# yemam3/SAC-RCBF

Measured on AMD Instinct MI355X. Metric: safe env steps/sec (dynamics+CBF-QP) at batch 65536, 1/2/4/8 MI355X, higher is better.
Workload: dtype f32 rows / f64 QP / f64 env

## Files before the change

__graft_entry__.py:

```python
import os
import subprocess
import sys

ROOT = os.path.dirname(os.path.abspath(__file__))
PKG = os.path.join(ROOT, "sac-rcbf_amd")
CSRC = os.path.join(PKG, "csrc")
LIB = os.path.join(PKG, "rcbf_amd", "librcbf_hip.so")
HIPCC = os.environ.get("HIPCC", "/opt/rocm/bin/hipcc")
HIP_FLAGS = ["--offload-arch=gfx950", "-O3", "-fPIC", "-std=c++17",
             "-fhip-fp32-correctly-rounded-divide-sqrt", "-Wno-unused-result",
             "-mllvm", "-amdgpu-kernarg-preload-count=16"]

for p in (ROOT, PKG):
    if p not in sys.path:
        sys.path.insert(0, p)


def _newer(target, sources):
    if not os.path.exists(target):
        return False
    t = os.path.getmtime(target)
    return all(os.path.getmtime(s) <= t for s in sources)


KERNEL_TUS = ["rcbf_qp.hip", "rcbf_qp_f64.hip", "rcbf_qp_bwd.hip", "rcbf_layer.hip", "rcbf_env.hip", "rcbf_cascade.hip",
              "rcbf_gp.hip", "rcbf_model.hip", "rcbf_aql.hip", "rcbf_steps_traj.hip", "rcbf_steps_term.hip"]
TU_FLAGS = {"rcbf_steps_term.hip": ["-mllvm", "-disable-machine-licm"]}
LLVM_BIN = "/opt/rocm/lib/llvm/bin"
STEPS_CO = os.path.join(PKG, "rcbf_amd", "librcbf_steps.co")
STEPS_TRAJ_CO = os.path.join(PKG, "rcbf_amd", "librcbf_steps_traj.co")
STEPS_TERM_CO = os.path.join(PKG, "rcbf_amd", "librcbf_steps_term.co")


def _deps(path, seen=None):
    import re
    seen = set() if seen is None else seen
    if path in seen or not os.path.exists(path):
        return seen
    seen.add(path)
    for name in re.findall(r'^\s*#\s*include\s+"([^"]+)"', open(path).read(), re.M):
        for d in (os.path.dirname(path), CSRC, os.path.join(ROOT, "include")):
            cand = os.path.normpath(os.path.join(d, name))
            if os.path.exists(cand):
                _deps(cand, seen)
                break
    return seen
# ... 13 lines not shown
        src = os.path.join(CSRC, tu)
        obj = os.path.join(objdir, tu.replace(".hip", ".o"))
        objs.append(obj)
        if not force and _newer(obj, sorted(_deps(src))):
            continue
        cmd = [HIPCC, *HIP_FLAGS, *TU_FLAGS.get(tu, []), *defines, *inc, "-c", "-o", obj, src]
        print("[build]", " ".join(cmd), flush=True)
        procs.append(subprocess.Popen(cmd))
    if any(p.wait() != 0 for p in procs):
        raise RuntimeError("hipcc failed")
    open(flags_file, "w").write(flags)
    if out == LIB:
        extract_steps_co(os.path.join(objdir, "rcbf_env.o"), STEPS_CO)
        extract_steps_co(os.path.join(objdir, "rcbf_steps_traj.o"), STEPS_TRAJ_CO)
        extract_steps_co(os.path.join(objdir, "rcbf_steps_term.o"), STEPS_TERM_CO)
    if not procs and _newer(out, objs):
        return out
    cmd = [HIPCC, "--offload-arch=gfx950", "-shared", "-fPIC", "-o", out, *objs, "-L/opt/rocm/lib", "-lhsa-runtime64"]
    print("[build]", " ".join(cmd), flush=True)
    subprocess.run(cmd, check=True)
    return out


def extract_steps_co(obj, out):
    if _newer(out, [obj]):
        return out
    import tempfile
    with tempfile.TemporaryDirectory() as td:
        fat = os.path.join(td, "fatbin.bin")
        subprocess.run([os.path.join(LLVM_BIN, "llvm-objcopy"), "--dump-section=.hip_fatbin=" + fat, obj,
# ... 139 lines not shown
    torch.cuda.synchronize()
    print("[smoke] ok", flush=True)


if __name__ == "__main__":
    what = sys.argv[1] if len(sys.argv) > 1 else "build"
    if what == "variant":
        name, defs = sys.argv[2], sys.argv[3:]
        os.makedirs(os.path.join(ROOT, "build", "variants"), exist_ok=True)
        vdir = os.path.join(ROOT, "build", "variants")
        build_lib(force=True, out=os.path.join(vdir, f"librcbf_{name}.so"), defines=defs)
        objdir = os.path.join(ROOT, "build", "obj_" + "_".join(d.strip("-D").replace("=", "") for d in defs))
        extract_steps_co(os.path.join(objdir, "rcbf_env.o"), os.path.join(vdir, f"librcbf_{name}.co"))
        extract_steps_co(os.path.join(objdir, "rcbf_steps_traj.o"), os.path.join(vdir, f"librcbf_{name}_traj.co"))
        extract_steps_co(os.path.join(objdir, "rcbf_steps_term.o"), os.path.join(vdir, f"librcbf_{name}_term.co"))
    else:
        {"build": build, "smoke": smoke, "build_oracle": lambda: build_oracle(force=True)}[what]()
```

include/rcbf_hip.h:

```cpp
#ifndef RCBF_HIP_H
#define RCBF_HIP_H

#include <stdint.h>
#include <hip/hip_runtime_api.h>

#ifdef __cplusplus
extern "C" {
#endif

#define RCBF_ABI_VERSION 13

#define RCBF_MODE_SIMULATED_CARS 0
#define RCBF_MODE_UNICYCLE 1

#define RCBF_FORM_DIFF 0
#define RCBF_FORM_CASCADE 1

#define RCBF_SOLVER_ACTIVE_SET 0
#define RCBF_SOLVER_PDIPM 1
#define RCBF_SOLVER_GI 2

#define RCBF_QP_OK 0
#define RCBF_QP_MAX_ITER 1
#define RCBF_QP_INFEASIBLE 2
// ... 221 lines not shown
#define RCBF_TRAJ_U 2
#define RCBF_TRAJ_REWARD 4
#define RCBF_TRAJ_COST 8
#define RCBF_TRAJ_DONE 16
#define RCBF_TRAJ_GOAL_MET 32
#define RCBF_TRAJ_STATUS 64
#define RCBF_TRAJ_TERM_OBS 128
#define RCBF_AQL_PROFILE 1
#define RCBF_AQL_FIRST_ACQUIRE_SYSTEM 2
#define RCBF_AQL_LAST_RELEASE_AGENT 4
#define RCBF_AQL_STUDY_MID_NOFENCE 8
#define RCBF_AQL_STUDY_MID_NOACQ 16
#define RCBF_AQL_STUDY_MID_NOREL 32
#define RCBF_AQL_PROFILE_ENDS 64
#define RCBF_AQL_PER_STEP 128
#define RCBF_AQL_SAFE_STEP_KERNARG_BYTES 408
#define RCBF_AQL_SAFE_STEPS_KERNARG_BYTES 408
#define RCBF_AQL_SAFE_STEPS_TRAJ_KERNARG_BYTES 424
#define RCBF_AQL_SAFE_STEPS_TERM_KERNARG_BYTES 432
typedef struct rcbf_aql rcbf_aql;
typedef struct rcbf_aql_plan rcbf_aql_plan;
int rcbf_aql_open(int32_t device, const char* code_object, int32_t flags, rcbf_aql** out);
int rcbf_aql_close(rcbf_aql* q);
int rcbf_aql_kernel_count(const rcbf_aql* q);
int rcbf_aql_safe_step_plan(rcbf_aql* q, const rcbf_params* prm, int64_t B, int32_t K, double* x, double* aux,
                            int32_t* step, uint32_t* episode, const float* const* u_rl_seq, int32_t n_u_rl,
                            const float* mu, const float* sigma, int32_t prior_cols, float* obs_out, float* u_out,
                            float* reward, float* cost, uint8_t* done, uint8_t* goal_met, int32_t* status_out,
                            int32_t* fail_flag, int32_t auto_reset, uint64_t seed, int64_t env_offset,
                            uint64_t* span_out, int32_t flags, rcbf_aql_plan** out);
// ... 2 lines not shown
                                 const float* mu, const float* sigma, int32_t prior_cols, float* obs_out,
                                 float* u_out, float* reward, float* cost, uint8_t* done, uint8_t* goal_met,
                                 int32_t* status_out, int32_t* fail_flag, int32_t auto_reset, uint64_t seed,
                                 int64_t env_offset, uint64_t* span_out, int32_t flags, int32_t traj_mask,
                                 int64_t traj_pitch, rcbf_aql_plan** out);
int rcbf_aql_safe_step_term_plan(rcbf_aql* q, const rcbf_params* prm, int64_t B, int32_t K, double* x, double* aux,
                                 int32_t* step, uint32_t* episode, const float* const* u_rl_seq, int32_t n_u_rl,
                                 const float* mu, const float* sigma, int32_t prior_cols, float* obs_out,
                                 float* u_out, float* reward, float* cost, uint8_t* done, uint8_t* goal_met,
                                 int32_t* status_out, int32_t* fail_flag, int32_t auto_reset, uint64_t seed,
                                 int64_t env_offset, uint64_t* span_out, int32_t flags, int32_t traj_mask,
                                 int64_t traj_pitch, float* term_obs, rcbf_aql_plan** out);
int rcbf_aql_run(rcbf_aql_plan* plan, uint64_t timeout_us);
int rcbf_aql_plan_times(const rcbf_aql_plan* plan, uint64_t* start_end_ns);
int rcbf_aql_plan_dispatches(const rcbf_aql_plan* plan);
int rcbf_aql_plan_free(rcbf_aql_plan* plan);

const char* rcbf_version(void);
int32_t rcbf_abi_version(void);
int32_t rcbf_params_size(void);

#ifdef __cplusplus
}
#endif
#endif
```

sac-rcbf_amd/csrc/rcbf_aql.hip:

```cpp
#include <hip/hip_runtime.h>
#include <hsa/hsa.h>
#include <hsa/hsa_ext_amd.h>

#include <dlfcn.h>
#include <immintrin.h>
#include <time.h>

#include <atomic>
#include <cstddef>
#include <cstdio>
#include <cstring>
#include <string>
#include <vector>

#include "rcbf_hip.h"
#include "rcbf_safe_step.hpp"

namespace {

using namespace rcbf;

struct SafeStepArgs {
    int64_t B;
    double* x;
// ... 49 lines not shown

}

struct rcbf_aql {
    int device = -1;
    hsa_agent_t agent{};
    hsa_queue_t* queue = nullptr;
    hsa_code_object_reader_t reader{};
    hsa_code_object_reader_t reader_traj{};
    hsa_executable_t exe{};
    hsa_executable_t exe_traj{};
    hsa_code_object_reader_t reader_term{};
    hsa_executable_t exe_term{};
    bool have_reader = false, have_reader_traj = false, have_exe = false, have_exe_traj = false, hsa_up = false;
    bool have_reader_term = false, have_exe_term = false;
    std::vector<char> code, code_traj, code_term;
    std::vector<KernelInfo> kernels;
    std::atomic<int> queue_error{0};
    int profiling = 0;
    bool fused = false;
    bool traj = false;
    bool term = false;
};

struct rcbf_aql_plan {
    rcbf_aql* q = nullptr;
    int device = -1;
    int32_t K = 0;
    void* kernargs = nullptr;
    std::vector<hsa_kernel_dispatch_packet_t> pkt;
    std::vector<hsa_signal_t> sig;
    int profiled = 0;
};

namespace {

void queue_error_cb(hsa_status_t status, hsa_queue_t*, void* data) {
    auto* q = static_cast<rcbf_aql*>(data);
    q->queue_error.store((int)status);
}

struct AgentSearch {
    uint32_t bdf;
    uint32_t domain;
    hsa_agent_t found{};
    bool ok = false;
};
// ... 49 lines not shown
    return buf;
}

std::string safe_steps_traj_prefix(int mode, int k, int bs) {
    char buf[128];
    snprintf(buf, sizeof buf, "_ZN4rcbf17k_safe_steps_trajILi%dELi%dELi%dEEEv", mode, k, bs);
    return buf;
}

std::string safe_steps_term_prefix(int mode, int k, int bs) {
    char buf[128];
    snprintf(buf, sizeof buf, "_ZN4rcbf17k_safe_steps_termILi%dELi%dELi%dEEEv", mode, k, bs);
    return buf;
}

bool read_side_code_object(const std::string& path, const char* suffix, std::vector<char>& code) {
    if (path.size() <= 3 || path.compare(path.size() - 3, 3, ".co") != 0) return true;
    const std::string tpath = path.substr(0, path.size() - 3) + suffix + ".co";
    FILE* tf = fopen(tpath.c_str(), "rb");
    if (!tf) return true;
    fseek(tf, 0, SEEK_END);
    const long tn = ftell(tf);
    fseek(tf, 0, SEEK_SET);
    code.resize(tn > 0 ? (size_t)tn : 0);
    const bool ok = tn > 0 && fread(code.data(), 1, (size_t)tn, tf) == (size_t)tn;
    fclose(tf);
    return ok;
}

template <typename T>
// ... 23 lines not shown
    explicit DeviceGuard(int dev) {
        if (hipGetDevice(&prev) != hipSuccess) prev = -1;
        if (prev != dev) (void)hipSetDevice(dev);
    }
    ~DeviceGuard() {
        if (prev >= 0) (void)hipSetDevice(prev);
    }
};

void destroy(rcbf_aql* q) {
    if (!q) return;
    if (q->queue) hsa_queue_destroy(q->queue);
    if (q->have_exe) hsa_executable_destroy(q->exe);
    if (q->have_exe_traj) hsa_executable_destroy(q->exe_traj);
    if (q->have_exe_term) hsa_executable_destroy(q->exe_term);
    if (q->have_reader) hsa_code_object_reader_destroy(q->reader);
    if (q->have_reader_traj) hsa_code_object_reader_destroy(q->reader_traj);
    if (q->have_reader_term) hsa_code_object_reader_destroy(q->reader_term);
    if (q->hsa_up) hsa_shut_down();
    delete q;
}

}

extern "C" {

int rcbf_aql_open(int32_t device, const char* code_object_path, int32_t flags, rcbf_aql** out) {
    if (!out) return RCBF_E_NULL;
    *out = nullptr;
    int ndev = 0;
    if (hipGetDeviceCount(&ndev) != hipSuccess || device < 0 || device >= ndev) return RCBF_E_BAD_SHAPE;
    std::string path;
    if (code_object_path && *code_object_path) {
// ... 13 lines not shown
    fseek(f, 0, SEEK_END);
    const long n = ftell(f);
    fseek(f, 0, SEEK_SET);
    q->code.resize(n > 0 ? (size_t)n : 0);
    const bool read_ok = n > 0 && fread(q->code.data(), 1, (size_t)n, f) == (size_t)n;
    fclose(f);
    if (!read_ok) {
        delete q;
        return RCBF_E_BAD_SHAPE;
    }
    if (!read_side_code_object(path, "_traj", q->code_traj)) {
        delete q;
        return RCBF_E_BAD_SHAPE;
    }
    if (!read_side_code_object(path, "_term", q->code_term)) {
        delete q;
        return RCBF_E_BAD_SHAPE;
    }
    int rc = hsa_rc(hsa_init());
    if (rc) {
        delete q;
        return rc;
    }
    q->hsa_up = true;
    hipDeviceProp_t prop;
    if (hipGetDeviceProperties(&prop, device) != hipSuccess) {
        destroy(q);
        return RCBF_E_HSA;
    }
    AgentSearch s{(uint32_t)((prop.pciBusID << 8) | (prop.pciDeviceID << 3)), (uint32_t)prop.pciDomainID};
// ... 28 lines not shown
    }
    if (!rc && !q->code_term.empty()) {
        rc = hsa_rc(
            hsa_code_object_reader_create_from_memory(q->code_term.data(), q->code_term.size(), &q->reader_term));
        if (!rc) q->have_reader_term = true;
        if (!rc)
            rc = hsa_rc(hsa_executable_create_alt(HSA_PROFILE_FULL, HSA_DEFAULT_FLOAT_ROUNDING_MODE_DEFAULT, nullptr,
                                                  &q->exe_term));
        if (!rc) q->have_exe_term = true;
        if (!rc)
            rc = hsa_rc(
                hsa_executable_load_agent_code_object(q->exe_term, q->agent, q->reader_term, nullptr, nullptr));
        if (!rc) rc = hsa_rc(hsa_executable_freeze(q->exe_term, nullptr));
        if (!rc) rc = hsa_rc(hsa_executable_iterate_agent_symbols(q->exe_term, q->agent, collect_kernel, q));
    }
    int n_steps = 0, n_fused = 0, n_traj = 0, n_term = 0;
    for (const auto& k : q->kernels) {
        if (k.name.compare(0, 21, "_ZN4rcbf11k_safe_step") == 0) {
            ++n_steps;
            if (k.kernarg_bytes != sizeof(SafeStepArgs) || k.private_bytes != 0) rc = RCBF_E_BAD_SHAPE;
        } else if (k.name.compare(0, 22, "_ZN4rcbf12k_safe_steps") == 0) {
            ++n_fused;
            if (k.kernarg_bytes != sizeof(SafeStepsArgs) || k.private_bytes != 0) rc = RCBF_E_BAD_SHAPE;
        } else if (k.name.compare(0, 27, "_ZN4rcbf17k_safe_steps_traj") == 0) {
            ++n_traj;
            if (k.kernarg_bytes != sizeof(SafeStepsTrajArgs) || k.private_bytes != 0) rc = RCBF_E_BAD_SHAPE;
        } else if (k.name.compare(0, 27, "_ZN4rcbf17k_safe_steps_term") == 0) {
            ++n_term;
            if (k.kernarg_bytes != sizeof(SafeStepsTermArgs) || k.private_bytes != 0) rc = RCBF_E_BAD_SHAPE;
        }
    }
    if (!rc && n_steps == 0) rc = RCBF_E_BAD_MODE;
    q->fused = n_fused > 0;
    q->traj = n_traj > 0;
    q->term = n_term > 0;
    if (!rc)
        rc = hsa_rc(hsa_queue_create(q->agent, kQueueSize, HSA_QUEUE_TYPE_SINGLE, queue_error_cb, q, UINT32_MAX,
                                     UINT32_MAX, &q->queue));
    if (!rc && q->profiling) rc = hsa_rc(hsa_amd_profiling_set_profiler_enabled(q->queue, 1));
    if (rc) {
        destroy(q);
        return rc;
    }
    *out = q;
    return 0;
}

int rcbf_aql_close(rcbf_aql* q) {
    destroy(q);
    return 0;
// ... 82 lines not shown
                       {reward, ext(row_rew, n * 4)},
                       {cost, ext(row_cost, n * 4)},
                       {done, ext(row_done, n)},
                       {goal_met, ext(row_goal, n)},
                       {status_out, ext(row_stat, n * 4)},
                       {term_obs, ext(row_term, 0)},
                       {fail_flag, 4}};
        for (int32_t j = 0; j < n_u_rl && kf; ++j)
            for (const auto& w : written)
                if (overlaps(u_rl_seq[j], nu * n * 4, w.p, w.bytes)) {
                    kf = nullptr;
                    break;
                }
    }
    if (term && !kf) return RCBF_E_BAD_MODE;
    const int32_t npkt = kf ? (K + kFusedChunk - 1) / kFusedChunk : K;

    auto* p = new rcbf_aql_plan();
    p->q = q;
    p->device = q->device;
    p->K = K;
    p->profiled = ends ? 2 : profiled ? 1 : 0;
    const size_t table_off = (size_t)npkt * kArgStride;
    std::vector<unsigned char> host(table_off + (kf ? (size_t)n_u_rl * sizeof(const float*) : 0), 0);
    int rc = (int)hipMalloc(&p->kernargs, host.size());
    if (kf) std::memcpy(host.data() + table_off, u_rl_seq, (size_t)n_u_rl * sizeof(const float*));
    for (int32_t j = 0; j < npkt && !rc; ++j) {
        const int64_t r0 = kf ? (int64_t)j * kFusedChunk : (int64_t)j;
        if (kf) {
            SafeStepsTermArgs ea;
            std::memset(&ea, 0, sizeof ea);
            SafeStepsTrajArgs& ta = ea.t;
            SafeStepsArgs& a = ta.s;
            ea.term_obs = rows_on(term_obs, r0, row_term);
            ta.traj_mask = traj_mask;
            ta.traj_pitch = traj_pitch;
            a.B = B;
// ... 49 lines not shown
        a.stamp_buf = span_out ? reinterpret_cast<unsigned long long*>(span_out) + (size_t)j * 4 * ((B + 63) / 64)
                               : nullptr;
        std::memcpy(host.data() + (size_t)j * kArgStride, &a, sizeof a);
    }
    if (!rc) rc = (int)hipMemcpy(p->kernargs, host.data(), host.size(), hipMemcpyHostToDevice);
    const int nsig = p->profiled == 1 ? npkt : p->profiled == 2 ? (npkt > 1 ? 2 : 1) : 1;
    for (int j = 0; !rc && j < nsig; ++j) {
        hsa_signal_t s;
        rc = hsa_rc(hsa_signal_create(1, 0, nullptr, &s));
        if (!rc) p->sig.push_back(s);
    }
    if (rc) {
        rcbf_aql_plan_free(p);
        return rc;
    }
    const KernelInfo* kd = kf ? kf : ki;
    p->pkt.resize(npkt);
    for (int32_t j = 0; j < npkt; ++j) {
        hsa_kernel_dispatch_packet_t& d = p->pkt[j];
        std::memset(&d, 0, sizeof d);
        int acq = j == 0 && (flags & RCBF_AQL_FIRST_ACQUIRE_SYSTEM) ? HSA_FENCE_SCOPE_SYSTEM : HSA_FENCE_SCOPE_AGENT;
        int rel =
            j == npkt - 1 && !(flags & RCBF_AQL_LAST_RELEASE_AGENT) ? HSA_FENCE_SCOPE_SYSTEM : HSA_FENCE_SCOPE_AGENT;
        if ((flags & (RCBF_AQL_STUDY_MID_NOFENCE | RCBF_AQL_STUDY_MID_NOACQ)) && j > 0) acq = HSA_FENCE_SCOPE_NONE;
        if ((flags & (RCBF_AQL_STUDY_MID_NOFENCE | RCBF_AQL_STUDY_MID_NOREL)) && j < npkt - 1)
            rel = HSA_FENCE_SCOPE_NONE;
        d.header = (uint16_t)((HSA_PACKET_TYPE_KERNEL_DISPATCH << HSA_PACKET_HEADER_TYPE) |
                              (1 << HSA_PACKET_HEADER_BARRIER) | (acq << HSA_PACKET_HEADER_SCACQUIRE_FENCE_SCOPE) |
                              (rel << HSA_PACKET_HEADER_SCRELEASE_FENCE_SCOPE));
        d.setup = (uint16_t)(1 << HSA_KERNEL_DISPATCH_PACKET_SETUP_DIMENSIONS);
        d.workgroup_size_x = (uint16_t)bs;
        d.workgroup_size_y = 1;
        d.workgroup_size_z = 1;
        d.grid_size_x = (uint32_t)(groups * (uint64_t)bs);
        d.grid_size_y = 1;
        d.grid_size_z = 1;
        d.private_segment_size = kd->private_bytes;
        d.group_segment_size = kd->group_bytes;
        d.kernel_object = kd->object;
        d.kernarg_address = static_cast<unsigned char*>(p->kernargs) + (size_t)j * kArgStride;
        if (p->profiled == 1)
            d.completion_signal = p->sig[j];
        else if (p->profiled == 2 && (j == 0 || j == npkt - 1))
            d.completion_signal = j == 0 ? p->sig.front() : p->sig.back();
        else if (j == npkt - 1)
            d.completion_signal = p->sig[0];
        else
            d.completion_signal.handle = 0;
    }
// ... 106 lines not shown
            start_end_ns[2 * j] = start_end_ns[2 * j + 1] = 0;
            if (j != 0 && j != p->K - 1) continue;
            sg = j == 0 ? p->sig.front() : p->sig.back();
        } else {
            sg = p->sig[j];
        }
        if (hsa_amd_profiling_get_dispatch_time(p->q->agent, sg, &t) != HSA_STATUS_SUCCESS) return RCBF_E_HSA;
        start_end_ns[2 * j] = (uint64_t)((long double)t.start * 1e9L / (long double)freq);
        start_end_ns[2 * j + 1] = (uint64_t)((long double)t.end * 1e9L / (long double)freq);
    }
    return 0;
}

int rcbf_aql_plan_dispatches(const rcbf_aql_plan* p) { return p ? (int)p->pkt.size() : RCBF_E_NULL; }

int rcbf_aql_plan_free(rcbf_aql_plan* p) {
    if (!p) return 0;
    if (p->kernargs) {
        DeviceGuard guard(p->device);
        (void)hipFree(p->kernargs);
    }
    for (auto& s : p->sig) hsa_signal_destroy(s);
    delete p;
    return 0;
}

}
```

sac-rcbf_amd/rcbf_amd/_lib.py:

```python
import ctypes
import os
import warnings

import torch

_HERE = os.path.dirname(os.path.abspath(__file__))
LIB_PATH = os.environ.get("RCBF_HIP_LIB", os.path.join(_HERE, "librcbf_hip.so"))

MODE_SIMULATED_CARS = 0
MODE_UNICYCLE = 1
FORM_DIFF = 0
FORM_CASCADE = 1
SOLVER_ACTIVE_SET = 0
SOLVER_PDIPM = 1
SOLVER_GI = 2
QP_OK, QP_MAX_ITER, QP_INFEASIBLE, QP_NONFINITE = 0, 1, 2, 3
MAX_HAZARDS = 8
ABI_VERSION = 13

_ERRORS = {1001: "RCBF_E_BAD_MODE", 1002: "RCBF_E_BAD_SHAPE", 1003: "RCBF_E_NULL", 1004: "RCBF_E_HSA",
           1005: "RCBF_E_TIMEOUT", 1006: "RCBF_E_GP_HANDOFF"}


class RcbfParams(ctypes.Structure):
# ... 87 lines not shown
                                _P, _P, _I32, _U64, _I64, _P, _I32, ctypes.POINTER(ctypes.c_void_p)],
    "rcbf_aql_safe_step_traj_plan": [_P, _PRM, _I64, _I32, _P, _P, _P, _P, _P, _I32, _P, _P, _I32, _P, _P, _P, _P, _P,
                                     _P, _P, _P, _I32, _U64, _I64, _P, _I32, _I32, _I64,
                                     ctypes.POINTER(ctypes.c_void_p)],
    "rcbf_aql_safe_step_term_plan": [_P, _PRM, _I64, _I32, _P, _P, _P, _P, _P, _I32, _P, _P, _I32, _P, _P, _P, _P, _P,
                                     _P, _P, _P, _I32, _U64, _I64, _P, _I32, _I32, _I64, _P,
                                     ctypes.POINTER(ctypes.c_void_p)],
    "rcbf_traj_pack_replay_f64": [_P, _I64, _I64, _I64, _I32, _I64, _I32, _I32, _P, _P, _P, _P, _P, _P, _P, _I32,
                                  ctypes.c_double, _I32, _P],
    "rcbf_traj_pack_gp_f64": [_P, _P, _P, _P, _I64, _I32, _I64, _I32, _I32, _P, _P, _P, _P, _P, _P, ctypes.c_double,
                              _I32, _I32, _I64, _P],
    "rcbf_traj_pack_gp_scratch_bytes": [_I64, _I32],
    "rcbf_aql_run": [_P, _U64],
    "rcbf_aql_plan_times": [_P, _P],
    "rcbf_aql_plan_dispatches": [_P],
    "rcbf_aql_plan_free": [_P],
    "rcbf_host_free": [_P],
    "rcbf_version": [],
    "rcbf_abi_version": [],
    "rcbf_params_size": [],
}

_lib = None
_load_error = None


def load():
    global _lib, _load_error
    if _lib is not None:
        return _lib
# ... 98 lines not shown
```

sac-rcbf_amd/rcbf_amd/aql.py:

```python
import ctypes
import weakref

import torch

from . import _lib

PROFILE = 1
PROFILE_ENDS = 64
PER_STEP = 128
TRAJ_OBS, TRAJ_U, TRAJ_REWARD, TRAJ_COST, TRAJ_DONE, TRAJ_GOAL_MET, TRAJ_STATUS = 1, 2, 4, 8, 16, 32, 64
TRAJ_BITS = {"obs": TRAJ_OBS, "u": TRAJ_U, "reward": TRAJ_REWARD, "cost": TRAJ_COST, "done": TRAJ_DONE,
             "goal_met": TRAJ_GOAL_MET, "status": TRAJ_STATUS}
TRAJ_TERM_OBS = 128


def _bind():
    return _lib.load()


def _check(rc, what):
    _lib.check(rc, what)


class AqlQueue:
# ... 16 lines not shown
    def handle(self):
        if not self._fin.alive:
            raise RuntimeError("the AQL queue is closed")
        return self._h

    def kernel_count(self):
        return int(_lib.load().rcbf_aql_kernel_count(self.handle))

    def close(self):
        for p in list(self._plans):
            p.free()
        self._fin()

    def safe_step_plan(self, env, u_rl_seq, layer, steps=None, mean=None, sigma=None, outputs=None,
                       auto_reset=True, prior_layout="rows", span=None, profile=False, fence_flags=0, fused=None,
                       trajectory=None):
        if env.device != self.device:
            raise ValueError(f"env on {env.device}, queue on {self.device}")
        o = outputs if outputs is not None else env.make_outputs()
        us = [env._u_arg(u) for u in u_rl_seq]
        if not us:
            raise ValueError("u_rl_seq is empty")
        K = len(us) if steps is None else int(steps)
        if prior_layout not in ("rows", "cols"):
            raise ValueError(f"prior_layout must be 'rows' or 'cols', got {prior_layout!r}")
        cols = prior_layout == "cols"
        if cols:
            if mean is not None and env.dynamics_mode == "SimulatedCars":
                raise ValueError("the cars CBF rows read no mean (diff_cbf_qp.py:298-299): pass mean=None")
            mean, sigma = env._prior_cols_arg(mean, "mean"), env._prior_cols_arg(sigma, "sigma")
        else:
            mean, sigma = env._prior_arg(mean, "mean"), env._prior_arg(sigma, "sigma")
        if span is not None:
            nw = (env.num_envs + 63) // 64
            if not (torch.is_tensor(span) and span.dtype == torch.int64 and span.device == env.device
                    and span.is_contiguous() and span.numel() >= 4 * nw * K):
                raise ValueError(f"span must be a contiguous int64 tensor of >= {4 * nw * K} entries "
                                 f"(K blocks of ceil(B / 64) x 4) on {env.device}")
        a = env._step_args(layer, o, auto_reset)
        arr = (ctypes.c_void_p * len(us))(*[u.data_ptr() for u in us])
        h = ctypes.c_void_p()
        flags = (PROFILE if profile else 0) | (PER_STEP if fused is False else 0) | int(fence_flags)
        head = (self.handle, ctypes.byref(layer._prm), env.num_envs, K, *[v or None for v in a[2:6]], arr, len(us),
                None if mean is None else mean.data_ptr(), None if sigma is None else sigma.data_ptr(), int(cols))
        tail = (*a[17:20], None if span is None else span.data_ptr(), flags)
        traj = None
        if trajectory is not None and trajectory is not False:
            if span is not None:
                raise ValueError("a trajectory plan takes no span buffer")
            traj = env.make_trajectory(K) if trajectory is True else dict(trajectory)
            mask, pitch = _trajectory_args(env, traj, K)
            term = traj.get("term_obs")
            if term is not None:
                why = _term_plan_refusal(env, layer, us, term, K, pitch, profile, fused, fence_flags)
                if why:
                    raise ValueError(f"a trajectory plan with term_obs is always fused, but {why}")
            outs = list(a[9:17])
# ... 85 lines not shown
            o = self._keep[2]
            for f, t in self.trajectory.items():
                if f == "term_obs":
                    continue
                dst = self._env.obs if f == "obs" else o.get(f)
                if dst is not None and not (f == "goal_met" and self._env.dynamics_mode == "SimulatedCars"):
                    dst.copy_(t[self.K - 1])
        return self._env.obs, self._keep[2]["reward"], self._keep[2]["done"], self._keep[2]

    @property
    def dispatches(self):
        if not self._fin.alive:
            raise RuntimeError("the AQL plan was freed")
        return int(_lib.load().rcbf_aql_plan_dispatches(self._h))

    def times_ns(self):
        import numpy as np
        if not self._fin.alive or not self.queue._fin.alive:
            raise RuntimeError("the AQL plan (or its queue) was freed")
        out = np.zeros((self.K, 2), dtype=np.uint64)
        _check(_lib.load().rcbf_aql_plan_times(self._h, out.ctypes.data), "rcbf_aql_plan_times")
        return out.astype(np.int64)

    def free(self):
        self._fin()
```

Measured before the change: 54.18 billion.

## Add warp-specialized split fused-steps kernel pipelining cars env and QP roles

Adds a fused multi-step kernel for the simulated-cars mode. Each workgroup runs two halves: one half advances the world cars and writes observations, the other solves the CBF-QP and steps the controlled car. The halves hand per-env data to each other through double-buffered LDS and meet at a barrier each step, so the env update of step n overlaps the QP of step n-1. The AQL planner picks this kernel when the wave count is small relative to the CU count, or when asked. In exchange it doubles the workgroup size, adds LDS use and a barrier per step, and only covers the cars mode without trajectory or term outputs.

```diff
diff --git a/__graft_entry__.py b/__graft_entry__.py
--- a/__graft_entry__.py
+++ b/__graft_entry__.py
@@ -24,12 +24,14 @@
 
 
 KERNEL_TUS = ["rcbf_qp.hip", "rcbf_qp_f64.hip", "rcbf_qp_bwd.hip", "rcbf_layer.hip", "rcbf_env.hip", "rcbf_cascade.hip",
-              "rcbf_gp.hip", "rcbf_model.hip", "rcbf_aql.hip", "rcbf_steps_traj.hip", "rcbf_steps_term.hip"]
+              "rcbf_gp.hip", "rcbf_model.hip", "rcbf_aql.hip", "rcbf_steps_traj.hip", "rcbf_steps_term.hip",
+              "rcbf_steps_split.hip"]
 TU_FLAGS = {"rcbf_steps_term.hip": ["-mllvm", "-disable-machine-licm"]}
 LLVM_BIN = "/opt/rocm/lib/llvm/bin"
 STEPS_CO = os.path.join(PKG, "rcbf_amd", "librcbf_steps.co")
 STEPS_TRAJ_CO = os.path.join(PKG, "rcbf_amd", "librcbf_steps_traj.co")
 STEPS_TERM_CO = os.path.join(PKG, "rcbf_amd", "librcbf_steps_term.co")
+STEPS_SPLIT_CO = os.path.join(PKG, "rcbf_amd", "librcbf_steps_split.co")
 
 
 def _deps(path, seen=None):
@@ -73,6 +75,7 @@
         extract_steps_co(os.path.join(objdir, "rcbf_env.o"), STEPS_CO)
         extract_steps_co(os.path.join(objdir, "rcbf_steps_traj.o"), STEPS_TRAJ_CO)
         extract_steps_co(os.path.join(objdir, "rcbf_steps_term.o"), STEPS_TERM_CO)
+        extract_steps_co(os.path.join(objdir, "rcbf_steps_split.o"), STEPS_SPLIT_CO)
     if not procs and _newer(out, objs):
         return out
     cmd = [HIPCC, "--offload-arch=gfx950", "-shared", "-fPIC", "-o", out, *objs, "-L/opt/rocm/lib", "-lhsa-runtime64"]
@@ -242,5 +245,6 @@
         extract_steps_co(os.path.join(objdir, "rcbf_env.o"), os.path.join(vdir, f"librcbf_{name}.co"))
         extract_steps_co(os.path.join(objdir, "rcbf_steps_traj.o"), os.path.join(vdir, f"librcbf_{name}_traj.co"))
         extract_steps_co(os.path.join(objdir, "rcbf_steps_term.o"), os.path.join(vdir, f"librcbf_{name}_term.co"))
+        extract_steps_co(os.path.join(objdir, "rcbf_steps_split.o"), os.path.join(vdir, f"librcbf_{name}_split.co"))
     else:
         {"build": build, "smoke": smoke, "build_oracle": lambda: build_oracle(force=True)}[what]()
diff --git a/include/rcbf_hip.h b/include/rcbf_hip.h
--- a/include/rcbf_hip.h
+++ b/include/rcbf_hip.h
@@ -259,6 +259,12 @@
 #define RCBF_AQL_STUDY_MID_NOREL 32
 #define RCBF_AQL_PROFILE_ENDS 64
 #define RCBF_AQL_PER_STEP 128
+#define RCBF_AQL_NO_SPLIT 256
+#define RCBF_AQL_STUDY_SPLIT_PAIR 512
+#define RCBF_AQL_SPLIT 1024
+#define RCBF_AQL_FORM_PER_STEP 0
+#define RCBF_AQL_FORM_FUSED 1
+#define RCBF_AQL_FORM_SPLIT 2
 #define RCBF_AQL_SAFE_STEP_KERNARG_BYTES 408
 #define RCBF_AQL_SAFE_STEPS_KERNARG_BYTES 408
 #define RCBF_AQL_SAFE_STEPS_TRAJ_KERNARG_BYTES 424
@@ -291,6 +297,7 @@
 int rcbf_aql_run(rcbf_aql_plan* plan, uint64_t timeout_us);
 int rcbf_aql_plan_times(const rcbf_aql_plan* plan, uint64_t* start_end_ns);
 int rcbf_aql_plan_dispatches(const rcbf_aql_plan* plan);
+int rcbf_aql_plan_form(const rcbf_aql_plan* plan);
 int rcbf_aql_plan_free(rcbf_aql_plan* plan);
 
 const char* rcbf_version(void);
diff --git a/sac-rcbf_amd/csrc/rcbf_aql.hip b/sac-rcbf_amd/csrc/rcbf_aql.hip
--- a/sac-rcbf_amd/csrc/rcbf_aql.hip
+++ b/sac-rcbf_amd/csrc/rcbf_aql.hip
@@ -87,13 +87,17 @@
     hsa_executable_t exe_term{};
     bool have_reader = false, have_reader_traj = false, have_exe = false, have_exe_traj = false, hsa_up = false;
     bool have_reader_term = false, have_exe_term = false;
-    std::vector<char> code, code_traj, code_term;
+    hsa_code_object_reader_t reader_split{};
+    hsa_executable_t exe_split{};
+    bool have_reader_split = false, have_exe_split = false;
+    std::vector<char> code, code_traj, code_term, code_split;
     std::vector<KernelInfo> kernels;
     std::atomic<int> queue_error{0};
     int profiling = 0;
     bool fused = false;
     bool traj = false;
     bool term = false;
+    bool split = false;
 };
 
 struct rcbf_aql_plan {
@@ -104,6 +108,7 @@
     std::vector<hsa_kernel_dispatch_packet_t> pkt;
     std::vector<hsa_signal_t> sig;
     int profiled = 0;
+    int form = RCBF_AQL_FORM_PER_STEP;
 };
 
 namespace {
@@ -183,6 +188,12 @@
     return buf;
 }
 
+std::string safe_steps_split_prefix(int bs) {
+    char buf[128];
+    snprintf(buf, sizeof buf, "_ZN4rcbf18k_safe_steps_splitILi%dEEEv", bs);
+    return buf;
+}
+
 bool read_side_code_object(const std::string& path, const char* suffix, std::vector<char>& code) {
     if (path.size() <= 3 || path.compare(path.size() - 3, 3, ".co") != 0) return true;
     const std::string tpath = path.substr(0, path.size() - 3) + suffix + ".co";
@@ -236,9 +247,11 @@
     if (q->have_exe) hsa_executable_destroy(q->exe);
     if (q->have_exe_traj) hsa_executable_destroy(q->exe_traj);
     if (q->have_exe_term) hsa_executable_destroy(q->exe_term);
+    if (q->have_exe_split) hsa_executable_destroy(q->exe_split);
     if (q->have_reader) hsa_code_object_reader_destroy(q->reader);
     if (q->have_reader_traj) hsa_code_object_reader_destroy(q->reader_traj);
     if (q->have_reader_term) hsa_code_object_reader_destroy(q->reader_term);
+    if (q->have_reader_split) hsa_code_object_reader_destroy(q->reader_split);
     if (q->hsa_up) hsa_shut_down();
     delete q;
 }
@@ -282,6 +295,10 @@
         return RCBF_E_BAD_SHAPE;
     }
     if (!read_side_code_object(path, "_term", q->code_term)) {
+        delete q;
+        return RCBF_E_BAD_SHAPE;
+    }
+    if (!read_side_code_object(path, "_split", q->code_split)) {
         delete q;
         return RCBF_E_BAD_SHAPE;
     }
@@ -340,7 +357,21 @@
         if (!rc) rc = hsa_rc(hsa_executable_freeze(q->exe_term, nullptr));
         if (!rc) rc = hsa_rc(hsa_executable_iterate_agent_symbols(q->exe_term, q->agent, collect_kernel, q));
     }
-    int n_steps = 0, n_fused = 0, n_traj = 0, n_term = 0;
+    if (!rc && !q->code_split.empty()) {
+        rc = hsa_rc(
+            hsa_code_object_reader_create_from_memory(q->code_split.data(), q->code_split.size(), &q->reader_split));
+        if (!rc) q->have_reader_split = true;
+        if (!rc)
+            rc = hsa_rc(hsa_executable_create_alt(HSA_PROFILE_FULL, HSA_DEFAULT_FLOAT_ROUNDING_MODE_DEFAULT, nullptr,
+                                                  &q->exe_split));
+        if (!rc) q->have_exe_split = true;
+        if (!rc)
+            rc = hsa_rc(
+                hsa_executable_load_agent_code_object(q->exe_split, q->agent, q->reader_split, nullptr, nullptr));
+        if (!rc) rc = hsa_rc(hsa_executable_freeze(q->exe_split, nullptr));
+        if (!rc) rc = hsa_rc(hsa_executable_iterate_agent_symbols(q->exe_split, q->agent, collect_kernel, q));
+    }
+    int n_steps = 0, n_fused = 0, n_traj = 0, n_term = 0, n_split = 0;
     for (const auto& k : q->kernels) {
         if (k.name.compare(0, 21, "_ZN4rcbf11k_safe_step") == 0) {
             ++n_steps;
@@ -354,12 +385,16 @@
         } else if (k.name.compare(0, 27, "_ZN4rcbf17k_safe_steps_term") == 0) {
             ++n_term;
             if (k.kernarg_bytes != sizeof(SafeStepsTermArgs) || k.private_bytes != 0) rc = RCBF_E_BAD_SHAPE;
+        } else if (k.name.compare(0, 28, "_ZN4rcbf18k_safe_steps_split") == 0) {
+            ++n_split;
+            if (k.kernarg_bytes != sizeof(SafeStepsArgs) || k.private_bytes != 0) rc = RCBF_E_BAD_SHAPE;
         }
     }
     if (!rc && n_steps == 0) rc = RCBF_E_BAD_MODE;
     q->fused = n_fused > 0;
     q->traj = n_traj > 0;
     q->term = n_term > 0;
+    q->split = n_split > 0;
     if (!rc)
         rc = hsa_rc(hsa_queue_create(q->agent, kQueueSize, HSA_QUEUE_TYPE_SINGLE, queue_error_cb, q, UINT32_MAX,
                                      UINT32_MAX, &q->queue));
@@ -472,6 +507,14 @@
                 }
     }
     if (term && !kf) return RCBF_E_BAD_MODE;
+    const bool pair = (flags & RCBF_AQL_STUDY_SPLIT_PAIR) != 0;
+    const bool split_asked = pair || (flags & RCBF_AQL_SPLIT) != 0;
+    const bool split_pays = 2 * ((B + 63) / 64) <= 4 * num_cus();
+    int sbs = pair ? 64 : bs;
+    const KernelInfo* ks = nullptr;
+    if (kf && cars && !traj_mask && !term && q->split && !(flags & RCBF_AQL_NO_SPLIT) && (split_asked || split_pays))
+        ks = find_kernel(q, safe_steps_split_prefix(sbs));
+    if (ks && ks->kernarg_bytes != sizeof(SafeStepsArgs)) ks = nullptr;
     const int32_t npkt = kf ? (K + kFusedChunk - 1) / kFusedChunk : K;
 
     auto* p = new rcbf_aql_plan();
@@ -479,6 +522,7 @@
     p->device = q->device;
     p->K = K;
     p->profiled = ends ? 2 : profiled ? 1 : 0;
+    p->form = ks ? RCBF_AQL_FORM_SPLIT : kf ? RCBF_AQL_FORM_FUSED : RCBF_AQL_FORM_PER_STEP;
     const size_t table_off = (size_t)npkt * kArgStride;
     std::vector<unsigned char> host(table_off + (kf ? (size_t)n_u_rl * sizeof(const float*) : 0), 0);
     int rc = (int)hipMalloc(&p->kernargs, host.size());
@@ -558,7 +602,9 @@
         rcbf_aql_plan_free(p);
         return rc;
     }
-    const KernelInfo* kd = kf ? kf : ki;
+    const KernelInfo* kd = ks ? ks : kf ? kf : ki;
+    const uint32_t wg = ks ? 2u * (uint32_t)sbs : (uint32_t)bs;
+    const uint64_t ngroups = ks ? (uint64_t)grid_for_envs(B, sbs) : groups;
     p->pkt.resize(npkt);
     for (int32_t j = 0; j < npkt; ++j) {
         hsa_kernel_dispatch_packet_t& d = p->pkt[j];
@@ -573,10 +619,10 @@
                               (1 << HSA_PACKET_HEADER_BARRIER) | (acq << HSA_PACKET_HEADER_SCACQUIRE_FENCE_SCOPE) |
                               (rel << HSA_PACKET_HEADER_SCRELEASE_FENCE_SCOPE));
         d.setup = (uint16_t)(1 << HSA_KERNEL_DISPATCH_PACKET_SETUP_DIMENSIONS);
-        d.workgroup_size_x = (uint16_t)bs;
+        d.workgroup_size_x = (uint16_t)wg;
         d.workgroup_size_y = 1;
         d.workgroup_size_z = 1;
-        d.grid_size_x = (uint32_t)(groups * (uint64_t)bs);
+        d.grid_size_x = (uint32_t)(ngroups * (uint64_t)wg);
         d.grid_size_y = 1;
         d.grid_size_z = 1;
         d.private_segment_size = kd->private_bytes;
@@ -713,6 +759,8 @@
 
 int rcbf_aql_plan_dispatches(const rcbf_aql_plan* p) { return p ? (int)p->pkt.size() : RCBF_E_NULL; }
 
+int rcbf_aql_plan_form(const rcbf_aql_plan* p) { return p ? p->form : RCBF_E_NULL; }
+
 int rcbf_aql_plan_free(rcbf_aql_plan* p) {
     if (!p) return 0;
     if (p->kernargs) {
diff --git a/sac-rcbf_amd/csrc/rcbf_steps_split.hip b/sac-rcbf_amd/csrc/rcbf_steps_split.hip
--- /dev/null
+++ b/sac-rcbf_amd/csrc/rcbf_steps_split.hip
@@ -0,0 +1,306 @@
+#include "rcbf_safe_step.hpp"
+
+namespace rcbf {
+
+__device__ __forceinline__ void cars_env_pre_world(const rcbf_params& prm, double* xs, double& t, int& step,
+                                                   bool& done) {
+#pragma clang fp contract(off)
+    const double kp = prm.kp, kb = prm.k_brake, dt = 0.02;
+    double vdes0 = 30.0 - 10.0 * sin_small(0.2 * t);
+    double acc[5];
+    acc[0] = kp * (vdes0 - xs[1]);
+#pragma unroll
+    for (int i = 1; i < 5; ++i)
+        if (i != 3) acc[i] = kp * (30.0 - xs[2 * i + 1]);
+    double d01 = xs[0] - xs[2], d12 = xs[2] - xs[4], d24 = xs[4] - xs[8];
+    acc[1] += (-kb * d01) * (d01 < 6.0 ? 1.0 : 0.0);
+    acc[2] += (-kb * d12) * (d12 < 6.0 ? 1.0 : 0.0);
+    acc[4] += (-kb * d24) * (d24 < 13.0 ? 1.0 : 0.0);
+#pragma unroll
+    for (int i = 0; i < 5; ++i)
+        if (i != 3) acc[i] *= 1.1;
+    double v[5];
+#pragma unroll
+    for (int i = 0; i < 5; ++i)
+        if (i != 3) v[i] = xs[2 * i + 1];
+#pragma unroll
+    for (int i = 0; i < 5; ++i) {
+        if (i != 3) {
+            xs[2 * i] += dt * v[i];
+            xs[2 * i + 1] += dt * acc[i];
+        }
+    }
+    t = t + dt;
+    step += 1;
+    done = step >= 300;
+}
+
+__device__ __forceinline__ double cars_env_pre_car3(const rcbf_params& prm, double* xs, double p2, double p4,
+                                                    double& cost_out) {
+#pragma clang fp contract(off)
+    const double kp = prm.kp, dt = 0.02;
+    double acc3 = kp * (30.0 - xs[7]);
+    acc3 *= 1.1;
+    const double v3 = xs[7];
+    xs[6] += dt * v3;
+    double cost = 0.0;
+    if (p2 - xs[6] < 2.99) cost -= 0.1;
+    if (xs[6] - p4 < 2.99) cost -= 0.1;
+    cost_out = cost;
+    return acc3;
+}
+
+__device__ __forceinline__ void split_barrier() {
+    asm volatile("" ::: "memory");
+    __builtin_amdgcn_s_waitcnt(0xc07f);
+    __builtin_amdgcn_s_barrier();
+    asm volatile("" ::: "memory");
+}
+
+__device__ __forceinline__ int auto_reset_from_kernargs() {
+    int v = 0;
+#if defined(__HIP_DEVICE_COMPILE__)
+    uint32_t zoff = 0;
+    asm volatile("" : "+s"(zoff));
+    typedef const char __attribute__((address_space(4)))* cbytes_t;
+    const cbytes_t ka = (cbytes_t)__builtin_amdgcn_kernarg_segment_ptr() + zoff;
+    v = *reinterpret_cast<const int32_t __attribute__((address_space(4)))*>(ka + offsetof(SafeStepsArgs, auto_reset));
+#endif
+    return v;
+}
+
+template <int BS>
+__global__ void __launch_bounds__(2 * BS) k_safe_steps_split(
+    int64_t B, double* __restrict__ x, double* __restrict__ aux, int32_t* __restrict__ step,
+    const float* const* __restrict__ u_tab, uint32_t* __restrict__ episode, const float* __restrict__ mu,
+    const float* __restrict__ sigma, float* __restrict__ obs_out, float* __restrict__ u_out,
+    float* __restrict__ reward, float* __restrict__ cost, uint8_t* __restrict__ done, uint8_t* __restrict__ goal_met,
+    int32_t* __restrict__ status_out, int32_t* fail_flag, int auto_reset, uint64_t seed, int64_t off, rcbf_params prm,
+    int prior_cols, int n_u, int steps, int ju0) {
+    constexpr int MODE = RCBF_MODE_SIMULATED_CARS, K = 1;
+    using D = Dims<MODE, K>;
+    constexpr int NW = BS / 64;
+    static_assert(BS % 64 == 0 && D::NO == 10 && D::NS == 10, "whole waves of cars");
+    (void)mu;
+    (void)auto_reset;
+    __shared__ float obs_stage[2][NW][64 * D::NO];
+    __shared__ float hand_o[2][5][BS];
+    __shared__ double hand_p[2][2][BS];
+    __shared__ int hand_dn[2][BS];
+    const int tid = threadIdx.x;
+    const bool role_b = __builtin_amdgcn_readfirstlane((int)(tid >= BS)) != 0;
+    const int le = tid & (BS - 1);
+    const int64_t i = (int64_t)blockIdx.x * BS + le;
+    const bool live = i < B;
+    const int lane = le & 63, wid = le >> 6;
+    const int64_t wbase = i - lane;
+    const gptr<double> xv = (gptr<double>)x;
+    const gptr<float> obsv = (gptr<float>)obs_out;
+    const bool full =
+        __builtin_amdgcn_readfirstlane((int)((wbase + 64 <= B) && ((reinterpret_cast<uintptr_t>(obs_out) & 15) == 0))) != 0;
+    const gptr<float> orow = obsv + i * D::NO;
+
+    if (!role_b) {
+        const gptr<double> auxv = (gptr<double>)aux;
+        const gptr<int32_t> stepv = (gptr<int32_t>)step;
+        const gptr<uint32_t> epv = (gptr<uint32_t>)episode;
+        const int ar = auto_reset_from_kernargs();
+        double xs[D::NS];
+#pragma unroll
+        for (int k = 0; k < D::NS; ++k) xs[k] = 0.0;
+        double a = 0.0;
+        int st = 0;
+        uint32_t epr = 0u;
+        if (live) {
+#pragma unroll
+            for (int p = 0; p < D::NS / 2; ++p) {
+                if (p == 3) continue;
+                typedef double d2 __attribute__((ext_vector_type(2)));
+                const d2 v = __builtin_nontemporal_load(reinterpret_cast<gptr<const d2>>(xv + 2 * (p * B + i)));
+                xs[2 * p] = v.x;
+                xs[2 * p + 1] = v.y;
+            }
+            a = ld_in((gptr<const double>)(auxv + i));
+            st = ld_in((gptr<const int32_t>)(stepv + i));
+            if (epv) epr = ld_in((gptr<const uint32_t>)(epv + i));
+        }
+        float oa[D::NO];
+        {
+            double o[D::NO];
+            env_obs<MODE>(xs, o);
+#pragma unroll
+            for (int k = 0; k < D::NO; ++k) oa[k] = (float)o[k];
+        }
+        __builtin_amdgcn_s_waitcnt(0x0f70);
+#pragma nounroll
+        for (int n = 0; n <= steps; ++n) {
+            const int par = n & 1;
+            if (n >= 2 && full)
+                store_obs_chunks<MODE, false, false, gptr<float>, false, true>(obsv, wbase, obs_stage[par][wid], lane);
+            if (live && n < steps) {
+                hand_o[par][0][le] = oa[2];
+                hand_o[par][1][le] = oa[4];
+                hand_o[par][2][le] = oa[5];
+                hand_o[par][3][le] = oa[8];
+                hand_o[par][4][le] = oa[9];
+                bool dn;
+                cars_env_pre_world(prm, xs, a, st, dn);
+                hand_p[par][0][le] = xs[4];
+                hand_p[par][1][le] = xs[8];
+                hand_dn[par][le] = (int)dn;
+                if (ar && dn) {
+                    const uint32_t ep = epv ? epr + 1u : 0u;
+                    if (epv) epv[i] = ep;
+                    env_reset_one<MODE>(nullptr, i, seed, off, ep, xs, a, st);
+                    epr += 1u;
+                }
+#pragma unroll
+                for (int p = 0; p < D::NS / 2; ++p)
+                    if (p != 3) st_out2d(xv + 2 * (p * B + i), xs[2 * p], xs[2 * p + 1]);
+                st_out(auxv + i, a);
+                st_out(stepv + i, (int32_t)st);
+                double o[D::NO];
+                env_obs<MODE>(xs, o);
+#pragma unroll
+                for (int k = 0; k < D::NO; ++k) oa[k] = (float)o[k];
+                if (full) {
+                    float* const row = &obs_stage[par][wid][lane * D::NO];
+#pragma unroll
+                    for (int k = 0; k < D::NO / 2; ++k)
+                        if (k != 3) *reinterpret_cast<float2*>(&row[2 * k]) = make_float2(oa[2 * k], oa[2 * k + 1]);
+                } else {
+#pragma unroll
+                    for (int k = 0; k < D::NO / 2; ++k)
+                        if (k != 3) st_out2(orow + 2 * k, oa[2 * k], oa[2 * k + 1]);
+                }
+            }
+            split_barrier();
+        }
+        if (steps >= 1 && full)
+            store_obs_chunks<MODE, false, false, gptr<float>, false, true>(obsv, wbase, obs_stage[(steps - 1) & 1][wid],
+                                                                           lane);
+        return;
+    }
+
+    const gptr<float> uv = (gptr<float>)u_out;
+    const gptr<float> rewv = (gptr<float>)reward;
+    const gptr<float> costv = (gptr<float>)cost;
+    const gptr<uint8_t> donev = (gptr<uint8_t>)done;
+    const gptr<uint8_t> goalv = (gptr<uint8_t>)goal_met;
+    const gptr<int32_t> statv = (gptr<int32_t>)status_out;
+    const gptr<int32_t> failv = (gptr<int32_t>)fail_flag;
+    const int ar = auto_reset_from_kernargs();
+    typedef const uint64_t __attribute__((address_space(4)))* ctab_t;
+    const ctab_t tab = (ctab_t)reinterpret_cast<const uint64_t*>(u_tab);
+    const gptr<const float> u0 = reinterpret_cast<gptr<const float>>(tab[ju0]);
+    int ju = ju0 + 1 == n_u ? 0 : ju0 + 1;
+    uint64_t unext = tab[ju];
+    double xs[D::NS];
+#pragma unroll
+    for (int k = 0; k < D::NS; ++k) xs[k] = 0.0;
+    float us[D::NU] = {0.0f}, m[D::NS], s[D::NS];
+#pragma unroll
+    for (int k = 0; k < D::NS; ++k) {
+        m[k] = 0.0f;
+        s[k] = prior_sigma<MODE>(k);
+    }
+    if (live) {
+        typedef double d2 __attribute__((ext_vector_type(2)));
+        const d2 v = __builtin_nontemporal_load(reinterpret_cast<gptr<const d2>>(xv + 2 * (3 * B + i)));
+        xs[6] = v.x;
+        xs[7] = v.y;
+        us[0] = ld_in(u0 + i);
+        const gptr<const float> sg = (gptr<const float>)sigma;
+        if (sg) {
+            if (prior_cols) {
+                s[5] = ld_in(sg + i);
+                s[7] = ld_in(sg + (B + i));
+                s[9] = ld_in(sg + (2 * B + i));
+            } else {
+                s[5] = ld_in(sg + (i * D::NS + 5));
+                s[7] = ld_in(sg + (i * D::NS + 7));
+                s[9] = ld_in(sg + (i * D::NS + 9));
+            }
+        }
+    }
+    float ob6, ob7;
+    {
+        double o[D::NO];
+        env_obs<MODE>(xs, o);
+        ob6 = (float)o[6];
+        ob7 = (float)o[7];
+    }
+    __builtin_amdgcn_s_waitcnt(0x0f70);
+#pragma nounroll
+    for (int n = 0; n <= steps; ++n) {
+        const int j = n - 1, par = j & 1;
+        uint64_t unext2 = unext;
+        if (n >= 1) {
+            ju = ju + 1 == n_u ? 0 : ju + 1;
+            unext2 = tab[ju];
+        }
+        if (live && n >= 1) {
+            float un = 0.0f;
+            if (n < steps) un = ld_in(reinterpret_cast<gptr<const float>>(unext) + i);
+            float oc[D::NO], s32[D::NS];
+#pragma unroll
+            for (int k = 0; k < D::NO; ++k) oc[k] = 0.0f;
+            oc[2] = hand_o[par][0][le];
+            oc[4] = hand_o[par][1][le];
+            oc[5] = hand_o[par][2][le];
+            oc[8] = hand_o[par][3][le];
+            oc[9] = hand_o[par][4][le];
+            oc[6] = ob6;
+            oc[7] = ob7;
+            const double p2 = hand_p[par][0][le], p4 = hand_p[par][1][le];
+            const bool dn = hand_dn[par][le] != 0;
+            state_from_obs32<MODE>(oc, s32);
+            LayerState<MODE, K> L;
+            diff_rows<MODE, K>(prm, s32, us, m, s, L.G, L.h, nullptr);
+            double cst_d;
+            const double acc3 = cars_env_pre_car3(prm, xs, p2, p4, cst_d);
+            const float cst = (float)cst_d;
+            float uf[D::NU];
+            layer_solve_raw<MODE, K>(prm, us, uf, L);
+            const int status = L.qp.status;
+            CarsStepOut o;
+            cars_env_post<float>(xs, acc3, uf[0], o);
+            if (ar && dn) {
+                double xr[D::NS];
+                cars_reset_state(xr, 0.0);
+                xs[6] = xr[6];
+                xs[7] = xr[7];
+            }
+            st_out2d(xv + 2 * (3 * B + i), xs[6], xs[7]);
+            double od[D::NO];
+            env_obs<MODE>(xs, od);
+            ob6 = (float)od[6];
+            ob7 = (float)od[7];
+            if (full)
+                *reinterpret_cast<float2*>(&obs_stage[par][wid][lane * D::NO + 6]) = make_float2(ob6, ob7);
+            else
+                st_out2(orow + 6, ob6, ob7);
+            st_out(uv + i, uf[0]);
+            st_out(rewv + i, o.reward);
+            st_out(costv + i, cst);
+            st_out(donev + i, (uint8_t)dn);
+            if (goalv) st_out(goalv + i, (uint8_t)0);
+            report(status, statv, i, failv);
+            us[0] = un;
+        }
+        unext = unext2;
+        split_barrier();
+    }
+}
+
+#define RCBF_SAFE_STEPS_SPLIT_INSTANTIATE(BS_)                                                                      \
+    template __global__ void k_safe_steps_split<BS_>(                                                               \
+        int64_t, double* __restrict__, double* __restrict__, int32_t* __restrict__, const float* const* __restrict__, \
+        uint32_t* __restrict__, const float* __restrict__, const float* __restrict__, float* __restrict__,          \
+        float* __restrict__, float* __restrict__, float* __restrict__, uint8_t* __restrict__, uint8_t* __restrict__, \
+        int32_t* __restrict__, int32_t*, int, uint64_t, int64_t, rcbf_params, int, int, int, int)
+RCBF_SAFE_STEPS_SPLIT_INSTANTIATE(64);
+RCBF_SAFE_STEPS_SPLIT_INSTANTIATE(128);
+RCBF_SAFE_STEPS_SPLIT_INSTANTIATE(256);
+
+}
diff --git a/sac-rcbf_amd/rcbf_amd/_lib.py b/sac-rcbf_amd/rcbf_amd/_lib.py
--- a/sac-rcbf_amd/rcbf_amd/_lib.py
+++ b/sac-rcbf_amd/rcbf_amd/_lib.py
@@ -125,6 +125,7 @@
     "rcbf_aql_run": [_P, _U64],
     "rcbf_aql_plan_times": [_P, _P],
     "rcbf_aql_plan_dispatches": [_P],
+    "rcbf_aql_plan_form": [_P],
     "rcbf_aql_plan_free": [_P],
     "rcbf_host_free": [_P],
     "rcbf_version": [],
diff --git a/sac-rcbf_amd/rcbf_amd/aql.py b/sac-rcbf_amd/rcbf_amd/aql.py
--- a/sac-rcbf_amd/rcbf_amd/aql.py
+++ b/sac-rcbf_amd/rcbf_amd/aql.py
@@ -8,6 +8,10 @@
 PROFILE = 1
 PROFILE_ENDS = 64
 PER_STEP = 128
+NO_SPLIT = 256
+STUDY_SPLIT_PAIR = 512
+SPLIT = 1024
+FORMS = ("per_step", "fused", "split")
 TRAJ_OBS, TRAJ_U, TRAJ_REWARD, TRAJ_COST, TRAJ_DONE, TRAJ_GOAL_MET, TRAJ_STATUS = 1, 2, 4, 8, 16, 32, 64
 TRAJ_BITS = {"obs": TRAJ_OBS, "u": TRAJ_U, "reward": TRAJ_REWARD, "cost": TRAJ_COST, "done": TRAJ_DONE,
              "goal_met": TRAJ_GOAL_MET, "status": TRAJ_STATUS}
@@ -54,7 +58,7 @@
 
     def safe_step_plan(self, env, u_rl_seq, layer, steps=None, mean=None, sigma=None, outputs=None,
                        auto_reset=True, prior_layout="rows", span=None, profile=False, fence_flags=0, fused=None,
-                       trajectory=None):
+                       trajectory=None, split=None):
         if env.device != self.device:
             raise ValueError(f"env on {env.device}, queue on {self.device}")
         o = outputs if outputs is not None else env.make_outputs()
@@ -80,7 +84,8 @@
         a = env._step_args(layer, o, auto_reset)
         arr = (ctypes.c_void_p * len(us))(*[u.data_ptr() for u in us])
         h = ctypes.c_void_p()
-        flags = (PROFILE if profile else 0) | (PER_STEP if fused is False else 0) | int(fence_flags)
+        flags = (PROFILE if profile else 0) | (PER_STEP if fused is False else 0) | \
+            (NO_SPLIT if split is False else SPLIT if split is True else 0) | int(fence_flags)
         head = (self.handle, ctypes.byref(layer._prm), env.num_envs, K, *[v or None for v in a[2:6]], arr, len(us),
                 None if mean is None else mean.data_ptr(), None if sigma is None else sigma.data_ptr(), int(cols))
         tail = (*a[17:20], None if span is None else span.data_ptr(), flags)
@@ -196,6 +201,12 @@
             raise RuntimeError("the AQL plan was freed")
         return int(_lib.load().rcbf_aql_plan_dispatches(self._h))
 
+    @property
+    def form(self):
+        if not self._fin.alive:
+            raise RuntimeError("the AQL plan was freed")
+        return FORMS[int(_lib.load().rcbf_aql_plan_form(self._h))]
+
     def times_ns(self):
         import numpy as np
         if not self._fin.alive or not self.queue._fin.alive:
```

Result: slower. 53.07 billion (-2.1%).
